# tsurumeso/vocal-remover

Measured on NVIDIA H100. Metric: seconds-of-audio/sec separated (n_fft=2048, hop=1024), higher is better.
Workload: dtype bf16x3 (split-bf16 operands hi+lo, 3 wgmma passes, fp32 accumulate); fft/lstm fp32

## Files before the change

### vocal-remover_b200/csrc/conv_tc.cu

```cuda
#include <cuda.h>
#include <stdio.h>

#include <map>
#include <tuple>

#include "engine.h"
#include "tc_common.cuh"
#include "tc_plan.h"

namespace vr {

static constexpr int kMaxStages = 8;
static constexpr int kConsumerWarps = 8;
static constexpr int kThreads = 32 * kConsumerWarps + 32;
static constexpr int kStaticSmem = 2048;

struct TcParams {
  int N, Ho, Wo, Wt, Ht, Nt, tiles_w, tiles_h, m_tiles, n_tiles;
  int stride, pad_h, pad_w, dil_h, dil_w, KW;
  int cchunks, total_sub, CinPadTC, Cout, act, stages;
  bf16* out_hi;
  bf16* out_lo;
  int64_t osn, osh;
  int osw;
  const float* bias;
};

template <int KB, int BN>
__global__ void __launch_bounds__(kThreads, 1)
    conv_tc_kernel(const __grid_constant__ CUtensorMap tmA, const __grid_constant__ CUtensorMap tmB, const TcParams p) {
  constexpr int SUBS = 64 / KB;
  constexpr int kSteps = KB / 16;
  constexpr uint32_t kAPlane = 128 * KB * 2;
  constexpr uint32_t kASub = 2 * kAPlane;
  constexpr uint32_t kBPlane = BN * KB * 2;
  constexpr uint32_t kBSub = 2 * kBPlane;
  constexpr uint32_t kStageBytes = SUBS * (kASub + kBSub);
  constexpr uint32_t kBRegion = SUBS * kASub;
  constexpr uint32_t kLayout = KB == 64 ? 1u : KB == 32 ? 2u : 3u;
  extern __shared__ uint8_t smem_raw[];
  __shared__ __align__(8) uint64_t bar_full[kMaxStages];
  __shared__ __align__(8) uint64_t bar_empty[kMaxStages];
  __shared__ float bias_s[256];

  const int warp = __shfl_sync(0xffffffffu, (int)threadIdx.x >> 5, 0);
  const int lane = threadIdx.x & 31;
  const uint32_t smem_base = (smem_u32(smem_raw) + 1023u) & ~1023u;
  const int total_tiles = p.m_tiles * p.n_tiles;
  const int num_iters = (p.total_sub + SUBS - 1) / SUBS;

  if (warp == kConsumerWarps && lane == 0) {
    tma_prefetch(&tmA);
    tma_prefetch(&tmB);
    MbarRing(smem_u32(&bar_full[0]), smem_u32(&bar_empty[0]), 0, p.stages).init(1, kConsumerWarps);
    asm volatile("fence.mbarrier_init.release.cluster;" ::: "memory");
  }
  for (int i = threadIdx.x; i < p.n_tiles * BN; i += blockDim.x) bias_s[i] = __ldg(p.bias + i);
  __syncthreads();

  if (warp == kConsumerWarps) {
    if (elect_one_sync()) {
      MbarRing ring(smem_u32(&bar_full[0]), smem_u32(&bar_empty[0]), 0, p.stages);
      for (int tile = blockIdx.x; tile < total_tiles; tile += gridDim.x) {
        const int nt = tile % p.n_tiles;
        const int mt = tile / p.n_tiles;
        const int w0 = (mt % p.tiles_w) * p.Wt;
        const int h0 = ((mt / p.tiles_w) % p.tiles_h) * p.Ht;
        const int n0 = (mt / (p.tiles_w * p.tiles_h)) * p.Nt;
        const int wbase = w0 * p.stride - p.pad_w, hbase = h0 * p.stride - p.pad_h;
        const int nrow = nt * BN;
        int cc = 0, kw = 0, kh = 0, sub = 0;
        for (int it = 0; it < num_iters; ++it) {
          ring.wait_empty();
          const int nsub = min(SUBS, p.total_sub - sub);
          const uint32_t full = ring.full();
          const uint32_t sbase = smem_base + (uint32_t)ring.slot * kStageBytes;
          mbar_expect_tx(full, (uint32_t)nsub * (kASub + kBSub));
#pragma unroll
          for (int j = 0; j < SUBS; ++j) {
            if (j < nsub) {
              tma_load_5d(sbase + (uint32_t)j * kASub, &tmA, cc * KB, wbase + kw * p.dil_w, hbase + kh * p.dil_h, n0, 0, full);
              tma_load_3d(sbase + kBRegion + (uint32_t)j * kBSub, &tmB, (kh * p.KW + kw) * p.CinPadTC + cc * KB, nrow, 0,
                          full);
              ++sub;
              if (++cc == p.cchunks) {
                cc = 0;
                if (++kw == p.KW) {
                  kw = 0;
                  ++kh;
                }
              }
            }
          }
          ring.advance();
        }
      }
    }
    __syncwarp();
  } else {
    const int wg = warp >> 2;
    const float slope = act_slope(p.act);
    const uint32_t dhi = desc_hi(8 * KB * 2, kLayout);
    MbarRing ring(smem_u32(&bar_full[0]), smem_u32(&bar_empty[0]), 0, p.stages);
    float acc[BN / 2];
    for (int tile = blockIdx.x; tile < total_tiles; tile += gridDim.x) {
#pragma unroll
      for (int i = 0; i < BN / 2; ++i) acc[i] = 0.f;
      HeldSlot held;
      for (int it = 0; it < num_iters; ++it) {
        const int nsub = min(SUBS, p.total_sub - it * SUBS);
        ring.wait_full();
        const uint32_t sdesc = desc_lo(smem_base + (uint32_t)ring.slot * kStageBytes);
        wg_fence();
#pragma unroll
        for (int j = 0; j < SUBS; ++j) {
          if (j < nsub) {
            const uint32_t a_hi = sdesc + ((j * kASub + (uint32_t)wg * (kAPlane / 2)) >> 4);
            const uint32_t a_lo = a_hi + (kAPlane >> 4);
            const uint32_t b_hi = sdesc + ((kBRegion + j * kBSub) >> 4);
            const uint32_t b_lo = b_hi + (kBPlane >> 4);
#pragma unroll
            for (int k = 0; k < kSteps; ++k)
              wgmma_split3<BN>(acc, a_hi + 2u * k, a_lo + 2u * k, b_hi + 2u * k, b_lo + 2u * k, dhi);
          }
        }
        wg_commit();
        wg_wait<1>();
        held.release(ring, lane);
        held.hold(ring);
        ring.advance();
      }
      wg_wait<0>();
      held.release_last(ring, lane);

      const int nt = tile % p.n_tiles;
      const int mt = tile / p.n_tiles;
      const int w0 = (mt % p.tiles_w) * p.Wt;
      const int h0 = ((mt / p.tiles_w) % p.tiles_h) * p.Ht;
      const int n0 = (mt / (p.tiles_w * p.tiles_h)) * p.Nt;
      const int c_lane = nt * BN + 2 * (lane & 3);
#pragma unroll
      for (int hr = 0; hr < 2; ++hr) {
        const int row = 64 * wg + 16 * (warp & 3) + (lane >> 2) + 8 * hr;
        const int dw = row % p.Wt;
        const int dh = (row / p.Wt) % p.Ht;
        const int n = n0 + row / (p.Wt * p.Ht);
        if (n >= p.N) continue;
        const int64_t obase = (int64_t)n * p.osn + (int64_t)(h0 + dh) * p.osh + (int64_t)(w0 + dw) * p.osw;
#pragma unroll
        for (int j = 0; j < BN / 8; ++j)
          epilogue_pair(acc[4 * j + 2 * hr], acc[4 * j + 2 * hr + 1], bias_s, c_lane + 8 * j, p.Cout, slope,
                        p.out_hi + obase, p.out_lo + obase);
      }
    }
  }
}

#define VR_TC_FOR_BN(X, KB) X(KB, 16) X(KB, 32) X(KB, 48) X(KB, 64) X(KB, 80) X(KB, 96) X(KB, 112) X(KB, 128)
#define VR_TC_FOR_ALL(X) VR_TC_FOR_BN(X, 64) VR_TC_FOR_BN(X, 32) VR_TC_FOR_BN(X, 16)


TcDebug g_debug;

static constexpr int kMaxDevices = 64;
const TcDevice& tc_device() {
  static TcDevice table[kMaxDevices];
  static TcDevice none;
  int dev = -1;
  if (cudaGetDevice(&dev) != cudaSuccess || dev < 0 || dev >= kMaxDevices) return none;
  TcDevice& d = table[dev];
  if (!d.ok) {
    if (cudaDeviceGetAttribute(&d.max_smem, cudaDevAttrMaxSharedMemoryPerBlockOptin, dev) != cudaSuccess ||
        cudaDeviceGetAttribute(&d.num_sms, cudaDevAttrMultiProcessorCount, dev) != cudaSuccess)
      return none;
#define VR_TC_SET_SMEM(KB, BN) \
  cudaFuncSetAttribute(conv_tc_kernel<KB, BN>, cudaFuncAttributeMaxDynamicSharedMemorySize, d.max_smem - kStaticSmem);
    VR_TC_FOR_ALL(VR_TC_SET_SMEM)
#undef VR_TC_SET_SMEM
    tc_rows_set_attributes(d.max_smem);
    tc_halo_set_attributes(d.max_smem);
    d.ok = true;
  }
  return d;
}

typedef CUresult (*EncodeTiledFn)(CUtensorMap*, CUtensorMapDataType, cuuint32_t, void*, const cuuint64_t*,
                                  const cuuint64_t*, const cuuint32_t*, const cuuint32_t*, CUtensorMapInterleave,
                                  CUtensorMapSwizzle, CUtensorMapL2promotion, CUtensorMapFloatOOBfill);
static EncodeTiledFn tc_encode_fn() {
  static EncodeTiledFn fn = nullptr;
  if (!fn) {
    void* p = nullptr;
    cudaDriverEntryPointQueryResult q;
    if (cudaGetDriverEntryPoint("cuTensorMapEncodeTiled", &p, cudaEnableDefault, &q) == cudaSuccess &&
        q == cudaDriverEntryPointSuccess)
      fn = (EncodeTiledFn)p;
  }
  return fn;
}

static CUtensorMapSwizzle swizzle_for(int KB) {
  return KB == 64 ? CU_TENSOR_MAP_SWIZZLE_128B : KB == 32 ? CU_TENSOR_MAP_SWIZZLE_64B : CU_TENSOR_MAP_SWIZZLE_32B;
}

static uint16_t tc_f2bf(float f) {
  uint32_t u;
  memcpy(&u, &f, 4);
  if ((u & 0x7fffffffu) > 0x7f800000u) return (uint16_t)((u >> 16) | 0x40);
  uint32_t r = 0x7fffu + ((u >> 16) & 1u);
  return (uint16_t)((u + r) >> 16);
}
static float tc_bf2f(uint16_t h) {
  uint32_t u = (uint32_t)h << 16;
  float f;
  memcpy(&f, &u, 4);
  return f;
}

struct TileGeom {
  int Wt, Ht, Nt;
  bool ok;
};
static TileGeom tile_geom(int Ho, int Wo) {
  TileGeom g{0, 0, 0, false};
  if (Wo <= 0 || Ho <= 0) return g;
  if (Wo >= 128) {
    if (Wo % 128) return g;
    g.Wt = 128; g.Ht = 1; g.Nt = 1;
  } else {
    if (128 % Wo) return g;
    g.Wt = Wo;
    g.Ht = 128 / Wo < Ho ? 128 / Wo : Ho;
    if (Ho % g.Ht) return g;
    if ((128 / Wo) % g.Ht) return g;
    g.Nt = 128 / (g.Wt * g.Ht);
  }
  g.ok = true;
  return g;
}

struct NTiling {
  int BN, n_tiles;
};
static NTiling n_tiling(const ConvLayer& L, bool rows, bool rows_wide) {
  const int cout16 = round_up(L.Cout, 16);
  if (rows) {
    const int BN = cout16 == 16 ? 16 : (rows_wide && cout16 % 64 == 0 ? 64 : 32);
    return {BN, ceil_div(cout16, BN)};
  }
  const int n_tiles = ceil_div(cout16, 128);
  return {round_up(ceil_div(cout16, n_tiles), 16), n_tiles};
}

TcKind tc_choose(const ConvLayer& L, int H, int W, bool rows_wide) {
  if (!(L.k == 1 || L.k == 3) || !(L.stride == 1 || L.stride == 2) || L.Cout < 4) return TC_NONE;
  const TileGeom g = tile_geom(H, W);
  if (!g.ok || g.Wt * L.stride > 256 || g.Ht * L.stride > 256) return TC_NONE;
  const bool k3s1 = L.k == 3 && L.stride == 1 && L.dil_h == 1 && L.dil_w == 1;
  const NTiling r = n_tiling(L, true, rows_wide), t = n_tiling(L, false, false);
  if (k3s1 && W % 128 == 0 && H % 8 == 0 && tc_rows_has(r.BN) && r.n_tiles * r.BN <= 256) return TC_ROWS;
  if (k3s1 && (W == 16 || W == 32 || W == 64) && H % (128 / W) == 0 && tc_halo_has(t.BN) &&
      t.n_tiles * t.BN <= 256 && g_debug.halo != 1)
    return TC_HALO;
  if (t.n_tiles * t.BN > 256) return TC_NONE;
  return TC_GENERIC;
}

template <class At>
static std::vector<uint16_t> split_bf16(const ConvLayer& L, const float* wp, int rows, int K, At at) {
  std::vector<uint16_t> planes((size_t)2 * rows * K, 0);
  const size_t lo = (size_t)rows * K;
  for (int co = 0; co < L.Cout; ++co)
    for (int t = 0; t < L.k * L.k; ++t)
      for (int ci = 0; ci < L.CinPad; ++ci) {
        const float w = wp[((size_t)t * L.CinPad + ci) * L.CoutPad + co];
        const uint16_t hi = tc_f2bf(w);
        const size_t i = at(co, t, ci);
        planes[i] = hi;
        planes[lo + i] = tc_f2bf(w - tc_bf2f(hi));
      }
  return planes;
}

static unsigned long long weight_group_mask(const ConvLayer& L, const float* wp, int CinPad) {
  if (CinPad / 8 > 64) return ~0ull;
  unsigned long long m = 0x3ull;
  for (int ci = 0; ci < L.CinPad; ++ci) {
    bool any = false;
    for (int t = 0; t < L.k * L.k && !any; ++t)
      for (int co = 0; co < L.Cout && !any; ++co) any = wp[((size_t)t * L.CinPad + ci) * L.CoutPad + co] != 0.f;
    if (any) m |= 1ull << (ci / 8);
  }
  return m;
}

static bool encode_weight_map(TcConv& tc, int rows, int K, int box_rows, std::string& err, const std::string& name) {
  cuuint64_t dims[3] = {(cuuint64_t)K, (cuuint64_t)rows, 2};
  cuuint64_t strides[2] = {(cuuint64_t)K * 2, (cuuint64_t)rows * K * 2};
  cuuint32_t box[3] = {(cuuint32_t)tc.KB, (cuuint32_t)box_rows, 2};
  cuuint32_t es[3] = {1, 1, 1};
  CUresult r = tc_encode_fn()(&tc.map_b, CU_TENSOR_MAP_DATA_TYPE_BFLOAT16, 3, tc.w_planes.get(), dims, strides, box, es,
                              CU_TENSOR_MAP_INTERLEAVE_NONE, swizzle_for(tc.KB), CU_TENSOR_MAP_L2_PROMOTION_L2_256B,
                              CU_TENSOR_MAP_FLOAT_OOB_FILL_NONE);
  if (r != CUDA_SUCCESS) {
    err = "cuTensorMapEncodeTiled(weights) failed for " + name + " code " + std::to_string((int)r);
    return false;
  }
  return true;
}

const CUtensorMap* tc_activation_map(TcConv& tc, const ActView& v, int bw, int bh, int bn, int es, std::string& err,
                                     const std::string& name) {
  const ViewKey key = std::make_tuple((const void*)v.hi, (const void*)v.lo, v.N, v.H, v.W, v.C, bw, bh, bn);
  auto it = tc.map_a.find(key);
  if (it != tc.map_a.end()) return &it->second;
  const int64_t plane = (const char*)v.lo - (const char*)v.hi;
  if (v.sw % 8 || v.sh % 8 || v.sn % 8 || (reinterpret_cast<uintptr_t>(v.hi) & 15) || plane <= 0 || plane % 16) {
    err = "internal: the input of " + name + " is not 16-byte aligned or its lo plane does not follow its hi plane";
    return nullptr;
  }
  cuuint64_t dims[5] = {(cuuint64_t)v.C, (cuuint64_t)v.W, (cuuint64_t)v.H, (cuuint64_t)v.N, 2};
  cuuint64_t strides[4] = {(cuuint64_t)v.sw * 2, (cuuint64_t)v.sh * 2, (cuuint64_t)v.sn * 2, (cuuint64_t)plane};
  cuuint32_t box[5] = {(cuuint32_t)tc.KB, (cuuint32_t)bw, (cuuint32_t)bh, (cuuint32_t)bn, 2};
  cuuint32_t estr[5] = {1, (cuuint32_t)es, (cuuint32_t)es, 1, 1};
  CUtensorMap m;
  CUresult r = tc_encode_fn()(&m, CU_TENSOR_MAP_DATA_TYPE_BFLOAT16, 5, (void*)v.hi, dims, strides, box, estr,
                              CU_TENSOR_MAP_INTERLEAVE_NONE, swizzle_for(tc.KB), CU_TENSOR_MAP_L2_PROMOTION_L2_256B,
                              CU_TENSOR_MAP_FLOAT_OOB_FILL_NONE);
  if (r != CUDA_SUCCESS) {
    err = "cuTensorMapEncodeTiled(activations) failed for " + name + " code " + std::to_string((int)r);
    return nullptr;
  }
  return &tc.map_a.emplace(key, m).first->second;
}

bool tc_prepare(ConvLayer& L, const float* w, const float* b, int H, int W, bool rows_wide, std::string& err) {
  const TcKind kind = tc_choose(L, H, W, rows_wide);
  if (kind == TC_NONE) return true;
  if (!tc_encode_fn()) {
    err = "cuTensorMapEncodeTiled is not available from the driver";
    return false;
  }
  auto tc = std::make_shared<TcConv>();
  tc->kind = kind;
  tc->H = H; tc->W = W;
  const NTiling nt = n_tiling(L, kind == TC_ROWS, rows_wide);
  const int BN = nt.BN, cin16 = round_up(L.CinPad, 16);
  tc->BN = BN; tc->n_tiles = nt.n_tiles;
  tc->KB = kind != TC_GENERIC ? 32 : cin16 % 64 == 0 ? 64 : cin16 % 32 == 0 ? 32 : 16;
  const int CinPad = round_up(L.CinPad, tc->KB);
  tc->CinPad = CinPad;
  tc->chunks = CinPad / tc->KB;
  tc->kmask = weight_group_mask(L, w, CinPad);
  const int rows = nt.n_tiles * BN;
  std::vector<uint16_t> planes;
  int brows, K;
  if (kind == TC_ROWS) {
    brows = 3 * rows;
    K = 3 * CinPad;
    planes = split_bf16(L, w, brows, K, [&](int co, int t, int ci) {
      return (size_t)(co / BN * 3 * BN + (2 - t / 3) * BN + co % BN) * K + (size_t)(t % 3) * CinPad + ci;
    });
  } else {
    brows = rows;
    K = L.k * L.k * CinPad;
    planes = split_bf16(L, w, brows, K, [&](int co, int t, int ci) { return (size_t)co * K + (size_t)t * CinPad + ci; });
  }
  std::vector<float> bias((size_t)rows, 0.f);
  for (int co = 0; co < L.Cout; ++co) bias[(size_t)co] = b[co];
  if (tc->w_planes.alloc(planes.size() * 2) != cudaSuccess || tc->bias.alloc(bias.size() * 4) != cudaSuccess) {
    err = "cudaMalloc failed while packing tensor-core weights for " + L.name;
    return false;
  }
  if (!upload(tc->w_planes.get(), planes.data(), planes.size() * 2, err) ||
      !upload(tc->bias.get(), bias.data(), bias.size() * 4, err) ||
      !encode_weight_map(*tc, brows, K, kind == TC_ROWS ? 3 * BN : BN, err, L.name))
    return false;
  L.tc = tc;
  return true;
}

cudaError_t tc_launch(const ConvLayer& L, const ActView& in, const ActView& out, cudaStream_t s, std::string& err,
                      const ConvFusion& f) {
  TcConv& tc = *L.tc;
  if (out.H != tc.H || out.W != tc.W || (in.H - 1) / L.stride + 1 != out.H || (in.W - 1) / L.stride + 1 != out.W) {
    err = "internal: " + L.name + " is launched on maps of another size than it was prepared for";
    return cudaErrorInvalidValue;
  }
  if (tc.kind == TC_ROWS) return tc_rows_launch(L, tc, in, out, s, err, f);
  if (!f.empty()) {
    err = "tc_launch: fused work is only implemented in the row-streaming kernel";
    return cudaErrorInvalidValue;
  }
  if (tc.kind == TC_HALO) return tc_halo_launch(L, tc, in, out, s, err);
  const TileGeom g = tile_geom(out.H, out.W);
  const CUtensorMap* map_a = tc_activation_map(tc, in, g.Wt * L.stride, g.Ht * L.stride, g.Nt, L.stride, err, L.name);
  if (!map_a) return cudaErrorInvalidValue;
  const int SUBS = 64 / tc.KB;
  TcParams p;
  p.N = out.N; p.Ho = out.H; p.Wo = out.W;
  p.Wt = g.Wt; p.Ht = g.Ht; p.Nt = g.Nt;
  p.tiles_w = out.W / g.Wt; p.tiles_h = out.H / g.Ht;
  p.m_tiles = p.tiles_w * p.tiles_h * ceil_div(out.N, g.Nt);
  p.n_tiles = tc.n_tiles;
  p.stride = L.stride; p.dil_h = L.dil_h; p.dil_w = L.dil_w;
  p.pad_h = L.dil_h * (L.k / 2); p.pad_w = L.dil_w * (L.k / 2);
  p.KW = L.k;
  p.cchunks = tc.chunks; p.total_sub = L.k * L.k * tc.chunks;
  p.CinPadTC = tc.CinPad; p.Cout = L.Cout; p.act = L.act;
  const int stage_bytes = SUBS * (2 * 128 * tc.KB * 2 + 2 * tc.BN * tc.KB * 2);
  const TcDevice& dv = tc_device();
  if (!dv.ok) {
    err = "tc_launch: cannot query the current device";
    return cudaErrorInvalidValue;
  }
  const int dyn = dv.max_smem - kStaticSmem;
  p.stages = (dyn - 1024) / stage_bytes;
  if (p.stages > kMaxStages) p.stages = kMaxStages;
  if (p.stages < 2) {
    err = "tc_launch: shared memory too small for two pipeline stages";
    return cudaErrorInvalidValue;
  }
  p.out_hi = out.hi; p.out_lo = out.lo;
  p.osn = out.sn; p.osh = out.sh; p.osw = out.sw;
  p.bias = tc.bias.get();
  const int total_tiles = p.m_tiles * p.n_tiles;
  const int grid = total_tiles < dv.num_sms ? total_tiles : dv.num_sms;
#define VR_TC_LAUNCH(KB_, BN_)                                                       \
  if (tc.KB == KB_ && tc.BN == BN_) {                                                \
    conv_tc_kernel<KB_, BN_><<<grid, kThreads, dyn, s>>>(*map_a, tc.map_b, p);       \
    return cudaGetLastError();                                                       \
  }
  VR_TC_FOR_ALL(VR_TC_LAUNCH)
#undef VR_TC_LAUNCH
  err = "tc_launch: no kernel instantiation for this channel tile";
  return cudaErrorInvalidValue;
}

}
```

### vocal-remover_b200/csrc/conv_tc_halo.cu

```cuda
#include <stdio.h>

#include "engine.h"
#include "tc_common.cuh"
#include "tc_plan.h"

namespace vr {

static constexpr int kConsumerWarps = 8;
static constexpr int kProducerWarps = 4;
static constexpr int kThreads = 32 * (kConsumerWarps + kProducerWarps);
static constexpr int kLaunchRegs = 168;
static constexpr int kConsumerRegs = 232;
static constexpr int kProducerRegs = 40;
static_assert(kConsumerWarps * kConsumerRegs + kProducerWarps * kProducerRegs <=
                  (kConsumerWarps + kProducerWarps) * kLaunchRegs,
              "setmaxnreg.inc would wait forever for registers the block does not own");
static constexpr int kStaticSmem = 2048;
static constexpr int kMaxHSlots = 4;
static constexpr int kMaxWStages = 18;
static constexpr uint32_t kKB = 32;
static constexpr uint32_t kRowB = kKB * 2;

template <int BN>
struct HaloGeom {
  static constexpr uint32_t kBPlane = BN * kRowB;
  static constexpr uint32_t kWStage = 2 * kBPlane;
};

struct HaloParams {
  int N, H, W, lw, Ht, Wb, tiles_h, n_tiles, total_tiles;
  int chunks, CinPadH, Cout, act;
  int n_hslots, n_wstages;
  uint32_t hplane, hslot;
  unsigned long long kmask;
  bf16* out_hi;
  bf16* out_lo;
  int64_t osn, osh;
  int osw;
  const float* bias;
};

struct HaloConsumer {
  MbarRing h, w;
  HeldSlot held_w;
};

template <int BN, int MB>
__device__ __forceinline__ void consume_halo(HaloConsumer& st, const HaloParams& p, float* acc,
                                             uint32_t (&fr)[2][MB * 8], const uint32_t* q0, uint32_t h_base,
                                             uint32_t w_base, uint32_t dhi, int lane) {
  typedef HaloGeom<BN> G;
  st.h.wait_full();
  const uint32_t slot = h_base + (uint32_t)st.h.slot * p.hslot;
#pragma unroll
  for (int t = 0; t < 9; ++t) {
    const int kh = t / 3, kw = t % 3;
#pragma unroll
    for (int ks = 0; ks < 2; ++ks) {
      uint32_t* f = fr[ks];
#pragma unroll
      for (int b = 0; b < MB; ++b) {
        const uint32_t q = q0[b] + (uint32_t)(kh * p.Wb + kw);
        const uint32_t a = slot + (q << 6) + ((((uint32_t)(2 * ks) + ((uint32_t)lane >> 4)) ^ ((q >> 1) & 3u)) << 4);
        ldsm_x4(f + 8 * b, a);
        ldsm_x4(f + 8 * b + 4, a + p.hplane);
      }
      if (ks == 0) st.w.wait_full();
      const uint32_t b_hi = desc_lo(w_base + (uint32_t)st.w.slot * G::kWStage) + (uint32_t)(ks * 32 >> 4);
      wg_fence();
#pragma unroll
      for (int b = 0; b < MB; ++b)
        wgmma_split3_rs<BN>(acc + b * (BN / 2), f + 8 * b, f + 8 * b + 4, b_hi, b_hi + (G::kBPlane >> 4), dhi);
      wg_commit();
      if (t == 8 && ks == 1) warp_arrive(st.h.empty(), lane);
      wg_wait<1>();
      st.held_w.release(st.w, lane);
    }
    st.held_w.hold(st.w);
    st.w.advance();
  }
  st.h.advance();
}

template <int BN, int MB>
__global__ void __launch_bounds__(kThreads, 1)
    conv_tc_halo_kernel(const __grid_constant__ CUtensorMap tmA, const __grid_constant__ CUtensorMap tmB,
                        const HaloParams p) {
  typedef HaloGeom<BN> G;
  extern __shared__ uint8_t smem_raw[];
  __shared__ __align__(8) uint64_t bar_hfull[kMaxHSlots];
  __shared__ __align__(8) uint64_t bar_hempty[kMaxHSlots];
  __shared__ __align__(8) uint64_t bar_wfull[kMaxWStages];
  __shared__ __align__(8) uint64_t bar_wempty[kMaxWStages];
  __shared__ float bias_s[256];

  const int warp = __shfl_sync(0xffffffffu, (int)threadIdx.x >> 5, 0);
  const int lane = threadIdx.x & 31;
  const uint32_t smem_base = (smem_u32(smem_raw) + 1023u) & ~1023u;
  const uint32_t h_base = smem_base;
  const uint32_t w_base = smem_base + (uint32_t)p.n_hslots * p.hslot;
  MbarRing hring(smem_u32(&bar_hfull[0]), smem_u32(&bar_hempty[0]), 0, p.n_hslots);
  MbarRing wring(smem_u32(&bar_wfull[0]), smem_u32(&bar_wempty[0]), 0, p.n_wstages);

  if (warp == kConsumerWarps && lane == 0) {
    tma_prefetch(&tmA);
    tma_prefetch(&tmB);
    hring.init(1, kConsumerWarps);
    wring.init(1, kConsumerWarps);
    asm volatile("fence.mbarrier_init.release.cluster;" ::: "memory");
  }
  for (int i = threadIdx.x; i < p.n_tiles * BN; i += blockDim.x) bias_s[i] = __ldg(p.bias + i);
  __syncthreads();

  if (warp >= kConsumerWarps) {
    setmaxnreg_dec<kProducerRegs>();
    if (warp == kConsumerWarps && elect_one_sync()) {
      for (int tile = blockIdx.x; tile < p.total_tiles; tile += gridDim.x) {
        const int nt = tile % p.n_tiles;
        const int mt = tile / p.n_tiles;
        const int h0 = (mt % p.tiles_h) * p.Ht;
        const int n = mt / p.tiles_h;
        for (int cc = 0; cc < p.chunks; ++cc) {
          if (!chunk_groups(p.kmask, cc)) continue;
          hring.wait_empty();
          mbar_expect_tx(hring.full(), p.hslot);
          tma_load_5d(h_base + (uint32_t)hring.slot * p.hslot, &tmA, cc * (int)kKB, -1, h0 - 1, n, 0, hring.full());
          hring.advance();
          for (int t = 0; t < 9; ++t) {
            wring.wait_empty();
            mbar_expect_tx(wring.full(), G::kWStage);
            tma_load_3d(w_base + (uint32_t)wring.slot * G::kWStage, &tmB, t * p.CinPadH + cc * (int)kKB, nt * BN, 0,
                        wring.full());
            wring.advance();
          }
        }
      }
    }
    __syncwarp();
  } else {
    setmaxnreg_inc<kConsumerRegs>();
    const int wg = warp >> 2;
    const float slope = act_slope(p.act);
    const uint32_t dhi = desc_hi(8 * kRowB, 2u);
    uint32_t q0[MB];
#pragma unroll
    for (int b = 0; b < MB; ++b) {
      const int px = 64 * (MB * wg + b) + 16 * (warp & 3) + (lane & 15);
      q0[b] = (uint32_t)((px >> p.lw) * p.Wb + (px & (p.W - 1)));
    }
    HaloConsumer st{hring, wring};
    float acc[MB * BN / 2];
    uint32_t fr[2][MB * 8];
    for (int tile = blockIdx.x; tile < p.total_tiles; tile += gridDim.x) {
#pragma unroll
      for (int i = 0; i < MB * BN / 2; ++i) acc[i] = 0.f;
      for (int cc = 0; cc < p.chunks; ++cc) {
        if (!chunk_groups(p.kmask, cc)) continue;
        consume_halo<BN, MB>(st, p, acc, fr, q0, h_base, w_base, dhi, lane);
      }
      wg_wait<0>();
      st.held_w.release_last(st.w, lane);

      const int nt = tile % p.n_tiles;
      const int mt = tile / p.n_tiles;
      const int h0 = (mt % p.tiles_h) * p.Ht;
      const int n = mt / p.tiles_h;
      const int c_lane = nt * BN + 2 * (lane & 3);
#pragma unroll
      for (int b = 0; b < MB; ++b) {
#pragma unroll
        for (int hr = 0; hr < 2; ++hr) {
          const int px = 64 * (MB * wg + b) + 16 * (warp & 3) + (lane >> 2) + 8 * hr;
          const int64_t obase =
              (int64_t)n * p.osn + (int64_t)(h0 + (px >> p.lw)) * p.osh + (int64_t)(px & (p.W - 1)) * p.osw;
          const float* v = acc + b * (BN / 2) + 2 * hr;
#pragma unroll
          for (int j = 0; j < BN / 8; ++j)
            epilogue_pair(v[4 * j], v[4 * j + 1], bias_s, c_lane + 8 * j, p.Cout, slope, p.out_hi + obase,
                          p.out_lo + obase);
        }
      }
    }
  }
}

#define VR_HALO_FOR_MB(X, BN) X(BN, 1) X(BN, 2)
#define VR_HALO_FOR_ALL(X) \
  VR_HALO_FOR_MB(X, 16) VR_HALO_FOR_MB(X, 32) VR_HALO_FOR_MB(X, 48) VR_HALO_FOR_MB(X, 64) VR_HALO_FOR_MB(X, 96) \
  VR_HALO_FOR_MB(X, 128)

bool tc_halo_has(int BN) {
#define VR_HALO_HAS(BN_, MB_) if (BN == BN_) return true;
  VR_HALO_FOR_ALL(VR_HALO_HAS)
#undef VR_HALO_HAS
  return false;
}

cudaError_t tc_halo_launch(const ConvLayer& L, TcConv& tc, const ActView& in, const ActView& out, cudaStream_t s,
                           std::string& err) {
  const TcDevice& dv = tc_device();
  if (!dv.ok) {
    err = "tc_halo_launch: cannot query the current device";
    return cudaErrorInvalidValue;
  }
  const int ht1 = 128 / out.W;
  const bool mb2_tiles = out.H % (2 * ht1) == 0;
  const int tiles1 = out.N * (out.H / ht1) * tc.n_tiles;
  const int waves1 = ceil_div(tiles1, dv.num_sms), waves2 = ceil_div(tiles1 / 2, dv.num_sms);
  int MB = mb2_tiles && 19 * waves2 <= 10 * waves1 ? 2 : 1;
  if (g_debug.halo == 2) MB = 1;
  if (g_debug.halo == 3 && mb2_tiles) MB = 2;
  HaloParams p;
  p.N = out.N; p.H = out.H; p.W = out.W;
  p.lw = out.W == 16 ? 4 : out.W == 32 ? 5 : 6;
  p.Ht = MB * ht1;
  p.Wb = round_up(out.W + 2, 8);
  p.tiles_h = out.H / p.Ht;
  p.n_tiles = tc.n_tiles;
  p.total_tiles = out.N * p.tiles_h * p.n_tiles;
  p.chunks = tc.chunks; p.CinPadH = tc.CinPad; p.Cout = L.Cout; p.act = L.act;
  p.hplane = (uint32_t)((p.Ht + 2) * p.Wb) * kRowB;
  p.hslot = 2 * p.hplane;
  p.kmask = g_debug.kskip == 1 ? tc.kmask : ~0ull;
  p.out_hi = out.hi; p.out_lo = out.lo;
  p.osn = out.sn; p.osh = out.sh; p.osw = out.sw;
  p.bias = tc.bias.get();
  const CUtensorMap* map_a = tc_activation_map(tc, in, p.Wb, p.Ht + 2, 1, 1, err, L.name);
  if (!map_a) return cudaErrorInvalidValue;
  const int w_stage = tc.BN * 2 * (int)kRowB;
  const int dyn = dv.max_smem - kStaticSmem;
  const int avail = dyn - 1024;
  p.n_hslots = (avail - 9 * w_stage) / (int)p.hslot;
  if (p.n_hslots > kMaxHSlots) p.n_hslots = kMaxHSlots;
  if (p.n_hslots < 2) p.n_hslots = 2;
  p.n_wstages = (avail - p.n_hslots * (int)p.hslot) / w_stage;
  if (p.n_wstages > kMaxWStages) p.n_wstages = kMaxWStages;
  if (p.n_wstages < 2) {
    err = "tc_halo_launch: shared memory too small for two halo slots and two weight stages";
    return cudaErrorInvalidValue;
  }
  const int grid = p.total_tiles < dv.num_sms ? p.total_tiles : dv.num_sms;
#define VR_HALO_LAUNCH(BN_, MB_)                                                        \
  if (tc.BN == BN_ && MB == MB_) {                                                      \
    conv_tc_halo_kernel<BN_, MB_><<<grid, kThreads, dyn, s>>>(*map_a, tc.map_b, p);     \
    return cudaGetLastError();                                                          \
  }
  VR_HALO_FOR_ALL(VR_HALO_LAUNCH)
#undef VR_HALO_LAUNCH
  err = "tc_halo_launch: no kernel instantiation for this channel tile";
  return cudaErrorInvalidValue;
}


void tc_halo_set_attributes(int max_smem) {
#define VR_HALO_SET(BN_, MB_) \
  cudaFuncSetAttribute(conv_tc_halo_kernel<BN_, MB_>, cudaFuncAttributeMaxDynamicSharedMemorySize, max_smem - kStaticSmem);
  VR_HALO_FOR_ALL(VR_HALO_SET)
#undef VR_HALO_SET
}

}
```

### vocal-remover_b200/csrc/tc_plan.h

```cpp
#pragma once
#include <cuda.h>

#include <map>
#include <tuple>

#include "engine.h"

namespace vr {

enum TcKind {
  TC_NONE,
  TC_GENERIC,
  TC_ROWS,
  TC_HALO,
};

typedef std::tuple<const void*, const void*, int, int, int, int, int, int, int> ViewKey;

struct TcConv {
  TcKind kind = TC_NONE;
  int H = 0, W = 0;
  int KB = 0, CinPad = 0, chunks = 0, BN = 0, n_tiles = 0;
  unsigned long long kmask = ~0ull;
  DevPtr<bf16> w_planes;
  DevPtr<float> bias;
  CUtensorMap map_b;
  std::map<ViewKey, CUtensorMap> map_a;
  bool fuses_upsample(int up_C) const { return kind == TC_ROWS && up_C % 32 == 0 && up_C <= CinPad; }
  bool fuses_dot() const { return kind == TC_ROWS; }
  bool fuses_mask(int Cout, int offset, bool up) const {
    const int kept = W - 2 * offset;
    return kind == TC_ROWS && up && n_tiles == 1 && BN <= 32 && BN == Cout && offset >= 0 && kept > 0 &&
           kept % 128 == 0;
  }
};

TcKind tc_choose(const ConvLayer& L, int H, int W, bool rows_wide);
const CUtensorMap* tc_activation_map(TcConv& tc, const ActView& v, int bw, int bh, int bn, int es, std::string& err,
                                     const std::string& name);

cudaError_t tc_rows_launch(const ConvLayer& L, TcConv& tc, const ActView& in, const ActView& out, cudaStream_t s,
                           std::string& err, const ConvFusion& f);
void tc_rows_set_attributes(int max_smem);
bool tc_rows_has(int BN);
int tc_rows_read_trace(unsigned long long* out, long long capacity);

cudaError_t tc_halo_launch(const ConvLayer& L, TcConv& tc, const ActView& in, const ActView& out, cudaStream_t s,
                           std::string& err);
void tc_halo_set_attributes(int max_smem);
bool tc_halo_has(int BN);

struct TcDevice {
  bool ok = false;
  int num_sms = 0, max_smem = 0;
};
const TcDevice& tc_device();

struct TcDebug {
  int trace = 0;
  int rows_wide = 0;
  int halo = 0;
  int kskip = 1;
  int crop_mask = 1;
};
extern TcDebug g_debug;

}
```

Measured before the change: 2859.

## Extend halo conv kernel to stride-2 3x3 convolutions and width tiling

Generalises the halo tensor-core convolution kernel with a compile-time stride parameter and tiling along width, so stride-2 3x3 layers (encoder downsampling) and W=128 inputs can use the halo path instead of the generic im2col-style kernel. The halo tile loaded by TMA covers the strided receptive field, and the A-operand offsets are scaled by the stride. The intent is to reuse each loaded input halo across all nine taps rather than re-fetching per tap. Stride-2 tiles load roughly four times the input footprint per output tile, and only MB=1 is instantiated for them, which raises shared-memory pressure and reduces pipeline depth.

```diff
diff --git a/vocal-remover_b200/csrc/conv_tc.cu b/vocal-remover_b200/csrc/conv_tc.cu
--- a/vocal-remover_b200/csrc/conv_tc.cu
+++ b/vocal-remover_b200/csrc/conv_tc.cu
@@ -256,12 +256,11 @@
   if (!(L.k == 1 || L.k == 3) || !(L.stride == 1 || L.stride == 2) || L.Cout < 4) return TC_NONE;
   const TileGeom g = tile_geom(H, W);
   if (!g.ok || g.Wt * L.stride > 256 || g.Ht * L.stride > 256) return TC_NONE;
-  const bool k3s1 = L.k == 3 && L.stride == 1 && L.dil_h == 1 && L.dil_w == 1;
+  const bool k3 = L.k == 3 && L.dil_h == 1 && L.dil_w == 1;
+  const bool k3s1 = k3 && L.stride == 1;
   const NTiling r = n_tiling(L, true, rows_wide), t = n_tiling(L, false, false);
   if (k3s1 && W % 128 == 0 && H % 8 == 0 && tc_rows_has(r.BN) && r.n_tiles * r.BN <= 256) return TC_ROWS;
-  if (k3s1 && (W == 16 || W == 32 || W == 64) && H % (128 / W) == 0 && tc_halo_has(t.BN) &&
-      t.n_tiles * t.BN <= 256 && g_debug.halo != 1)
-    return TC_HALO;
+  if (k3 && tc_halo_tiles(L.stride, H, W, t.BN) && t.n_tiles * t.BN <= 256 && g_debug.halo != 1) return TC_HALO;
   if (t.n_tiles * t.BN > 256) return TC_NONE;
   return TC_GENERIC;
 }
diff --git a/vocal-remover_b200/csrc/conv_tc_halo.cu b/vocal-remover_b200/csrc/conv_tc_halo.cu
--- a/vocal-remover_b200/csrc/conv_tc_halo.cu
+++ b/vocal-remover_b200/csrc/conv_tc_halo.cu
@@ -28,7 +28,7 @@
 };
 
 struct HaloParams {
-  int N, H, W, lw, Ht, Wb, tiles_h, n_tiles, total_tiles;
+  int N, H, Wt, lw, Ht, Wb, tiles_h, n_tiles, total_tiles;
   int chunks, CinPadH, Cout, act;
   int n_hslots, n_wstages;
   uint32_t hplane, hslot;
@@ -37,6 +37,7 @@
   bf16* out_lo;
   int64_t osn, osh;
   int osw;
+  int tiles_w;
   const float* bias;
 };
 
@@ -82,10 +83,24 @@
   st.h.advance();
 }
 
-template <int BN, int MB>
-__global__ void __launch_bounds__(kThreads, 1)
-    conv_tc_halo_kernel(const __grid_constant__ CUtensorMap tmA, const __grid_constant__ CUtensorMap tmB,
-                        const HaloParams p) {
+struct HaloTile {
+  int nt, n, h0, w0;
+};
+template <int S>
+__device__ __forceinline__ HaloTile halo_tile(const HaloParams& p, int tile) {
+  HaloTile t;
+  t.nt = tile % p.n_tiles;
+  int mt = tile / p.n_tiles;
+  const int tiles_w = S == 1 ? 1 : p.tiles_w;
+  t.w0 = (mt % tiles_w) * p.Wt;
+  mt /= tiles_w;
+  t.h0 = (mt % p.tiles_h) * p.Ht;
+  t.n = mt / p.tiles_h;
+  return t;
+}
+
+template <int BN, int MB, int S>
+__device__ __forceinline__ void halo_conv(const CUtensorMap& tmA, const CUtensorMap& tmB, const HaloParams& p) {
   typedef HaloGeom<BN> G;
   extern __shared__ uint8_t smem_raw[];
   __shared__ __align__(8) uint64_t bar_hfull[kMaxHSlots];
@@ -116,20 +131,18 @@
     setmaxnreg_dec<kProducerRegs>();
     if (warp == kConsumerWarps && elect_one_sync()) {
       for (int tile = blockIdx.x; tile < p.total_tiles; tile += gridDim.x) {
-        const int nt = tile % p.n_tiles;
-        const int mt = tile / p.n_tiles;
-        const int h0 = (mt % p.tiles_h) * p.Ht;
-        const int n = mt / p.tiles_h;
+        const HaloTile ot = halo_tile<S>(p, tile);
         for (int cc = 0; cc < p.chunks; ++cc) {
           if (!chunk_groups(p.kmask, cc)) continue;
           hring.wait_empty();
           mbar_expect_tx(hring.full(), p.hslot);
-          tma_load_5d(h_base + (uint32_t)hring.slot * p.hslot, &tmA, cc * (int)kKB, -1, h0 - 1, n, 0, hring.full());
+          tma_load_5d(h_base + (uint32_t)hring.slot * p.hslot, &tmA, cc * (int)kKB, S * ot.w0 - 1, S * ot.h0 - 1, ot.n,
+                      0, hring.full());
           hring.advance();
           for (int t = 0; t < 9; ++t) {
             wring.wait_empty();
             mbar_expect_tx(wring.full(), G::kWStage);
-            tma_load_3d(w_base + (uint32_t)wring.slot * G::kWStage, &tmB, t * p.CinPadH + cc * (int)kKB, nt * BN, 0,
+            tma_load_3d(w_base + (uint32_t)wring.slot * G::kWStage, &tmB, t * p.CinPadH + cc * (int)kKB, ot.nt * BN, 0,
                         wring.full());
             wring.advance();
           }
@@ -146,7 +159,7 @@
 #pragma unroll
     for (int b = 0; b < MB; ++b) {
       const int px = 64 * (MB * wg + b) + 16 * (warp & 3) + (lane & 15);
-      q0[b] = (uint32_t)((px >> p.lw) * p.Wb + (px & (p.W - 1)));
+      q0[b] = (uint32_t)(S * (px >> p.lw) * p.Wb + S * (px & (p.Wt - 1)));
     }
     HaloConsumer st{hring, wring};
     float acc[MB * BN / 2];
@@ -161,18 +174,15 @@
       wg_wait<0>();
       st.held_w.release_last(st.w, lane);
 
-      const int nt = tile % p.n_tiles;
-      const int mt = tile / p.n_tiles;
-      const int h0 = (mt % p.tiles_h) * p.Ht;
-      const int n = mt / p.tiles_h;
-      const int c_lane = nt * BN + 2 * (lane & 3);
+      const HaloTile ot = halo_tile<S>(p, tile);
+      const int c_lane = ot.nt * BN + 2 * (lane & 3);
 #pragma unroll
       for (int b = 0; b < MB; ++b) {
 #pragma unroll
         for (int hr = 0; hr < 2; ++hr) {
           const int px = 64 * (MB * wg + b) + 16 * (warp & 3) + (lane >> 2) + 8 * hr;
-          const int64_t obase =
-              (int64_t)n * p.osn + (int64_t)(h0 + (px >> p.lw)) * p.osh + (int64_t)(px & (p.W - 1)) * p.osw;
+          const int64_t obase = (int64_t)ot.n * p.osn + (int64_t)(ot.h0 + (px >> p.lw)) * p.osh +
+                                (int64_t)(ot.w0 + (px & (p.Wt - 1))) * p.osw;
           const float* v = acc + b * (BN / 2) + 2 * hr;
 #pragma unroll
           for (int j = 0; j < BN / 8; ++j)
@@ -184,16 +194,72 @@
   }
 }
 
-#define VR_HALO_FOR_MB(X, BN) X(BN, 1) X(BN, 2)
-#define VR_HALO_FOR_ALL(X) \
-  VR_HALO_FOR_MB(X, 16) VR_HALO_FOR_MB(X, 32) VR_HALO_FOR_MB(X, 48) VR_HALO_FOR_MB(X, 64) VR_HALO_FOR_MB(X, 96) \
-  VR_HALO_FOR_MB(X, 128)
-
-bool tc_halo_has(int BN) {
-#define VR_HALO_HAS(BN_, MB_) if (BN == BN_) return true;
+template <int BN, int MB>
+__global__ void __launch_bounds__(kThreads, 1)
+    conv_tc_halo_kernel(const __grid_constant__ CUtensorMap tmA, const __grid_constant__ CUtensorMap tmB,
+                        const HaloParams p) {
+  halo_conv<BN, MB, 1>(tmA, tmB, p);
+}
+template <int BN>
+__global__ void __launch_bounds__(kThreads, 1)
+    conv_tc_halo_s2_kernel(const __grid_constant__ CUtensorMap tmA, const __grid_constant__ CUtensorMap tmB,
+                           const HaloParams p) {
+  halo_conv<BN, 1, 2>(tmA, tmB, p);
+}
+
+typedef void (*HaloKernel)(const CUtensorMap, const CUtensorMap, const HaloParams);
+template <int BN, int MB, int S>
+static HaloKernel halo_kernel() {
+  if constexpr (S == 1)
+    return conv_tc_halo_kernel<BN, MB>;
+  else
+    return conv_tc_halo_s2_kernel<BN>;
+}
+
+#define VR_HALO_FOR_BN(X, BN) X(BN, 1, 1) X(BN, 2, 1)
+#define VR_HALO_FOR_ALL(X)                                                                                         \
+  VR_HALO_FOR_BN(X, 16) VR_HALO_FOR_BN(X, 32) VR_HALO_FOR_BN(X, 48) VR_HALO_FOR_BN(X, 64) VR_HALO_FOR_BN(X, 96)    \
+  VR_HALO_FOR_BN(X, 128) X(32, 1, 2) X(48, 1, 2) X(64, 1, 2)
+
+static bool halo_has(int BN, int S) {
+#define VR_HALO_HAS(BN_, MB_, S_) if (BN == BN_ && S == S_) return true;
   VR_HALO_FOR_ALL(VR_HALO_HAS)
 #undef VR_HALO_HAS
   return false;
+}
+
+struct HaloShape {
+  int Wt, lw, Ht, Wb;
+  uint32_t hplane;
+};
+static HaloShape halo_shape(int S, int W, int MB) {
+  HaloShape g;
+  g.Wt = W < 64 ? W : 64;
+  g.lw = g.Wt == 16 ? 4 : g.Wt == 32 ? 5 : 6;
+  g.Ht = 128 * MB / g.Wt;
+  g.Wb = round_up((g.Wt - 1) * S + 3, 8);
+  g.hplane = (uint32_t)(((g.Ht - 1) * S + 3) * g.Wb) * kRowB;
+  return g;
+}
+
+static bool halo_smem(int max_smem, uint32_t hslot, int BN, int& n_hslots, int& n_wstages) {
+  const int w_stage = BN * 2 * (int)kRowB;
+  const int avail = max_smem - kStaticSmem - 1024;
+  n_hslots = (avail - 9 * w_stage) / (int)hslot;
+  if (n_hslots > kMaxHSlots) n_hslots = kMaxHSlots;
+  if (n_hslots < 2) n_hslots = 2;
+  n_wstages = (avail - n_hslots * (int)hslot) / w_stage;
+  if (n_wstages > kMaxWStages) n_wstages = kMaxWStages;
+  return n_wstages >= 2;
+}
+
+bool tc_halo_tiles(int stride, int H, int W, int BN) {
+  if (!halo_has(BN, stride) || !(W == 16 || W == 32 || W == 64 || (stride == 2 && W == 128))) return false;
+  if (!(stride == 1 || stride == 2)) return false;
+  const HaloShape g = halo_shape(stride, W, 1);
+  const TcDevice& dv = tc_device();
+  int n_hslots, n_wstages;
+  return H % g.Ht == 0 && dv.ok && halo_smem(dv.max_smem, 2 * g.hplane, BN, n_hslots, n_wstages);
 }
 
 cudaError_t tc_halo_launch(const ConvLayer& L, TcConv& tc, const ActView& in, const ActView& out, cudaStream_t s,
@@ -203,58 +269,56 @@
     err = "tc_halo_launch: cannot query the current device";
     return cudaErrorInvalidValue;
   }
-  const int ht1 = 128 / out.W;
-  const bool mb2_tiles = out.H % (2 * ht1) == 0;
-  const int tiles1 = out.N * (out.H / ht1) * tc.n_tiles;
+  const int S = L.stride;
+  const HaloShape g1 = halo_shape(S, out.W, 1);
+  const bool mb2_tiles = S == 1 && out.H % (2 * g1.Ht) == 0;
+  const int tiles1 = out.N * (out.H / g1.Ht) * (out.W / g1.Wt) * tc.n_tiles;
   const int waves1 = ceil_div(tiles1, dv.num_sms), waves2 = ceil_div(tiles1 / 2, dv.num_sms);
   int MB = mb2_tiles && 19 * waves2 <= 10 * waves1 ? 2 : 1;
   if (g_debug.halo == 2) MB = 1;
   if (g_debug.halo == 3 && mb2_tiles) MB = 2;
+  const HaloShape g = halo_shape(S, out.W, MB);
   HaloParams p;
-  p.N = out.N; p.H = out.H; p.W = out.W;
-  p.lw = out.W == 16 ? 4 : out.W == 32 ? 5 : 6;
-  p.Ht = MB * ht1;
-  p.Wb = round_up(out.W + 2, 8);
+  p.N = out.N; p.H = out.H; p.Wt = g.Wt;
+  p.lw = g.lw;
+  p.Ht = g.Ht;
+  p.Wb = g.Wb;
   p.tiles_h = out.H / p.Ht;
+  p.tiles_w = out.W / p.Wt;
   p.n_tiles = tc.n_tiles;
-  p.total_tiles = out.N * p.tiles_h * p.n_tiles;
+  p.total_tiles = out.N * p.tiles_h * p.tiles_w * p.n_tiles;
   p.chunks = tc.chunks; p.CinPadH = tc.CinPad; p.Cout = L.Cout; p.act = L.act;
-  p.hplane = (uint32_t)((p.Ht + 2) * p.Wb) * kRowB;
+  p.hplane = g.hplane;
   p.hslot = 2 * p.hplane;
   p.kmask = g_debug.kskip == 1 ? tc.kmask : ~0ull;
   p.out_hi = out.hi; p.out_lo = out.lo;
   p.osn = out.sn; p.osh = out.sh; p.osw = out.sw;
   p.bias = tc.bias.get();
-  const CUtensorMap* map_a = tc_activation_map(tc, in, p.Wb, p.Ht + 2, 1, 1, err, L.name);
+  const CUtensorMap* map_a = tc_activation_map(tc, in, p.Wb, (p.Ht - 1) * S + 3, 1, 1, err, L.name);
   if (!map_a) return cudaErrorInvalidValue;
-  const int w_stage = tc.BN * 2 * (int)kRowB;
-  const int dyn = dv.max_smem - kStaticSmem;
-  const int avail = dyn - 1024;
-  p.n_hslots = (avail - 9 * w_stage) / (int)p.hslot;
-  if (p.n_hslots > kMaxHSlots) p.n_hslots = kMaxHSlots;
-  if (p.n_hslots < 2) p.n_hslots = 2;
-  p.n_wstages = (avail - p.n_hslots * (int)p.hslot) / w_stage;
-  if (p.n_wstages > kMaxWStages) p.n_wstages = kMaxWStages;
-  if (p.n_wstages < 2) {
+  if (!halo_smem(dv.max_smem, p.hslot, tc.BN, p.n_hslots, p.n_wstages)) {
     err = "tc_halo_launch: shared memory too small for two halo slots and two weight stages";
     return cudaErrorInvalidValue;
   }
+  const int dyn = dv.max_smem - kStaticSmem;
   const int grid = p.total_tiles < dv.num_sms ? p.total_tiles : dv.num_sms;
-#define VR_HALO_LAUNCH(BN_, MB_)                                                        \
-  if (tc.BN == BN_ && MB == MB_) {                                                      \
-    conv_tc_halo_kernel<BN_, MB_><<<grid, kThreads, dyn, s>>>(*map_a, tc.map_b, p);     \
-    return cudaGetLastError();                                                          \
+#define VR_HALO_LAUNCH(BN_, MB_, S_)                                          \
+  if (tc.BN == BN_ && MB == MB_ && S == S_) {                                 \
+    const HaloKernel kernel = halo_kernel<BN_, MB_, S_>();                     \
+    kernel<<<grid, kThreads, dyn, s>>>(*map_a, tc.map_b, p);                  \
+    return cudaGetLastError();                                                \
   }
   VR_HALO_FOR_ALL(VR_HALO_LAUNCH)
 #undef VR_HALO_LAUNCH
-  err = "tc_halo_launch: no kernel instantiation for this channel tile";
+  err = "tc_halo_launch: no kernel instantiation for this channel tile and stride";
   return cudaErrorInvalidValue;
 }
 
 
 void tc_halo_set_attributes(int max_smem) {
-#define VR_HALO_SET(BN_, MB_) \
-  cudaFuncSetAttribute(conv_tc_halo_kernel<BN_, MB_>, cudaFuncAttributeMaxDynamicSharedMemorySize, max_smem - kStaticSmem);
+#define VR_HALO_SET(BN_, MB_, S_)                                                                                 \
+  cudaFuncSetAttribute(halo_kernel<BN_, MB_, S_>(), cudaFuncAttributeMaxDynamicSharedMemorySize,                  \
+                       max_smem - kStaticSmem);
   VR_HALO_FOR_ALL(VR_HALO_SET)
 #undef VR_HALO_SET
 }
diff --git a/vocal-remover_b200/csrc/tc_plan.h b/vocal-remover_b200/csrc/tc_plan.h
--- a/vocal-remover_b200/csrc/tc_plan.h
+++ b/vocal-remover_b200/csrc/tc_plan.h
@@ -48,7 +48,7 @@
 cudaError_t tc_halo_launch(const ConvLayer& L, TcConv& tc, const ActView& in, const ActView& out, cudaStream_t s,
                            std::string& err);
 void tc_halo_set_attributes(int max_smem);
-bool tc_halo_has(int BN);
+bool tc_halo_tiles(int stride, int H, int W, int BN);
 
 struct TcDevice {
   bool ok = false;
```

Measured after the change: 2872, median of 6. About the same (+0.5%).
